# MisEty/RTG-SLAM

Measured on AMD Instinct MI355X. Metric: hot_path_units_per_sec, higher is better.
Workload: dtype f32; 1 GPU; `value` counts UNITS, not SLAM frames (the SLAM frame rate by the reference's definition is `slam_frames_per_sec`, from the `slam_sequence` leg of --full).  One UNIT per step = 1 ICP track (3 levels x 5 GN iters, 1200x680, on a second HIP stream) + 1 map-optimisation iteration (raster fwd + masked L1 colour / gated depth loss + attach regulariser + raster bwd + fused Adam) over 1200000 random Gaus; gaussians=1200000, mode=single, parallelism=1 GPU

## Files before the change

include/rtgs_debug.h:

```cpp
#ifndef RTGS_DEBUG_H
#define RTGS_DEBUG_H
#include "rtgs_raster.h"
#ifdef __cplusplus
extern "C" {
#endif

void rtgs_raster_set_counters(void* counters);
void rtgs_raster_set_counters_ctx(rtgs_ctx* ctx, void* counters);

void rtgs_raster_set_profiling(int enable);
void rtgs_raster_set_profiling_ctx(rtgs_ctx* ctx, int enable);

void rtgs_raster_set_near_slice(int mode, int budget_per_tile);
void rtgs_raster_set_near_slice_ctx(rtgs_ctx* ctx, int mode, int budget_per_tile);

void rtgs_raster_force_sort_path(int enable);
void rtgs_raster_force_sort_path_ctx(rtgs_ctx* ctx, int enable);
int rtgs_raster_last_timings(float* ms12_host);
int rtgs_raster_last_timings_ctx(rtgs_ctx* ctx, float* ms12_host);

void rtgs_raster_set_bwd_walk_ctx(rtgs_ctx* ctx, int mode);
void rtgs_raster_set_onepass_ctx(rtgs_ctx* ctx, int on);
void rtgs_raster_set_bwd_debug(int bits);
void rtgs_raster_set_bwd_stamps(void* dev);
void rtgs_raster_set_fwd_stamps(void* dev);
#define RTGS_ICP_STAMP_LAUNCHES 16
#define RTGS_ICP_STAMP_WGS 256
void rtgs_icp_set_stamps(void* dev);

#ifdef __cplusplus
}
#endif
#endif
```

rtg_slam_amd/_lib.py:

```python
from __future__ import annotations

import ctypes as C
import os
import threading

_HERE = os.path.dirname(os.path.abspath(__file__))
LIB_PATH = os.environ.get("RTGS_LIB_PATH") or os.path.join(_HERE, "librtgs_hip.so")

RESIZE_FN = C.CFUNCTYPE(C.c_void_p, C.c_void_p, C.c_size_t)
FWD_NO_BACKWARD = 1


class RasterSettingsC(C.Structure):
    _fields_ = [
        ("image_height", C.c_int32), ("image_width", C.c_int32),
        ("tanfovx", C.c_float), ("tanfovy", C.c_float),
        ("bg", C.c_void_p), ("scale_modifier", C.c_float),
        ("viewmatrix", C.c_void_p), ("projmatrix", C.c_void_p),
        ("sh_degree", C.c_int32), ("campos", C.c_void_p),
        ("opaque_threshold", C.c_float), ("depth_threshold", C.c_float),
        ("normal_threshold", C.c_float), ("color_sigma", C.c_float),
        ("prefiltered", C.c_int32), ("debug", C.c_int32),
        ("cx", C.c_float), ("cy", C.c_float), ("T_threshold", C.c_float),
    ]
# ... 93 lines not shown
    "rtgs_slam_loss_grads": (C.c_int, [_P, _P, _P, _P, _P, C.c_int32, C.c_int32, C.POINTER(LossCfgC), _P, _P, _P, _P, _P]),
    "rtgs_raster_set_profiling": (None, [C.c_int]),
    "rtgs_raster_force_sort_path": (None, [C.c_int]),
    "rtgs_raster_set_near_slice": (None, [C.c_int, C.c_int]),
    "rtgs_raster_last_slice_stats": (C.c_int, [C.POINTER(C.c_int64)]),
    "rtgs_raster_last_timings": (C.c_int, [C.POINTER(C.c_float)]),
    "rtgs_ctx_create": (C.c_void_p, []),
    "rtgs_ctx_destroy": (None, [_P]),
    "rtgs_raster_forward_ctx": (C.c_int, [_P, C.POINTER(RasterSettingsC), C.c_int32, C.c_int32] + [_P] * 6 + [_P]
                                + [_P] * 8 + [RESIZE_FN, _P, RESIZE_FN, _P, RESIZE_FN, _P, C.POINTER(C.c_int64),
                                              C.c_int32, _P]),
    "rtgs_raster_backward_ctx": (C.c_int, [_P, C.POINTER(RasterSettingsC), C.c_int32, C.c_int32, C.c_int64] + [_P] * 6
                                 + [_P] * 3 + [_P, _P, _P] + [_P, _P] + [_P] * 6 + [_P, _P]),
    "rtgs_raster_backward_rows_ctx": (C.c_int, [_P, C.POINTER(RasterSettingsC), C.c_int32, C.c_int32, C.c_int64] + [_P] * 6
                                      + [_P] * 3 + [_P, _P, _P] + [_P, _P] + [_P] * 6 + [_P, _P, _P]),
    "rtgs_raster_backward_range_ctx": (C.c_int, [_P, C.POINTER(RasterSettingsC), C.c_int32, C.c_int32, C.c_int64] + [_P] * 6
                                       + [_P] * 3 + [_P, _P, _P] + [_P, _P] + [_P] * 6 + [_P, _P, C.c_int32, C.c_int32, _P]),
    "rtgs_slam_normal_loss_range": (C.c_int, [_P, _P, _P, _P, C.c_int32, C.c_int32, C.c_float, _P, _P, _P, _P, _P,
                                              C.c_int32, C.c_int32, _P]),
    "rtgs_slam_normal_loss_sums": (C.c_int, [_P, _P, _P, _P, C.c_int32, C.c_int32, _P, _P, _P]),
    "rtgs_slam_normal_loss_grads": (C.c_int, [_P, _P, _P, _P, C.c_int32, C.c_int32, C.c_float, _P, _P, _P, _P, _P,
                                              C.c_int32, C.c_int32, _P]),
    "rtgs_raster_geom_bytes_ctx": (C.c_size_t, [_P, C.c_int32, C.c_int32, C.c_int32]),
    "rtgs_raster_last_stats_ctx": (C.c_int, [_P, C.POINTER(C.c_int64)]),
    "rtgs_raster_set_counters_ctx": (None, [_P, _P]),
    "rtgs_raster_set_profiling_ctx": (None, [_P, C.c_int]),
    "rtgs_raster_force_sort_path_ctx": (None, [_P, C.c_int]),
    "rtgs_raster_set_bwd_walk_ctx": (None, [_P, C.c_int]),
    "rtgs_raster_set_bwd_debug": (None, [C.c_int]),
    "rtgs_raster_set_bwd_stamps": (None, [C.c_void_p]),
    "rtgs_raster_set_fwd_stamps": (None, [C.c_void_p]),
    "rtgs_icp_set_stamps": (None, [C.c_void_p]),
    "rtgs_raster_set_onepass_ctx": (None, [_P, C.c_int]),
    "rtgs_raster_forward_verify_ctx": (C.c_int, [_P, C.POINTER(C.c_int64)]),
    "rtgs_raster_spec_fail_ptr_ctx": (C.c_void_p, [_P]),
    "rtgs_raster_set_speculation_ctx": (None, [_P, C.c_int]),
    "rtgs_raster_speculation_stats_ctx": (C.c_int, [_P, C.POINTER(C.c_int64)]),
    "rtgs_raster_plain_stats_ctx": (C.c_int, [_P, C.POINTER(C.c_int64)]),
    "rtgs_raster_set_plain_onepass_ctx": (None, [_P, C.c_int]),
    "rtgs_raster_image_offsets": (C.c_int, [C.c_int32, C.c_int32, C.POINTER(C.c_size_t)]),
    "rtgs_raster_set_near_slice_ctx": (None, [_P, C.c_int, C.c_int]),
    "rtgs_raster_last_slice_stats_ctx": (C.c_int, [_P, C.POINTER(C.c_int64)]),
    "rtgs_raster_last_timings_ctx": (C.c_int, [_P, C.POINTER(C.c_float)]),
    "rtgs_slam_map_step_ctx": (C.c_int, [_P, C.POINTER(MapStepArgsC), C.POINTER(C.c_int64), _P]),
    "rtgs_slam_map_step_front_ctx": (C.c_int, [_P, C.POINTER(MapStepArgsC), C.POINTER(C.c_int64), _P]),
    "rtgs_icp_build_pyramids": (C.c_int, [_P, C.c_int32, C.c_int32, _P, C.c_int32, C.POINTER(_P), C.POINTER(_P), _P, _P]),
    "rtgs_icp_build_pyramids_ex": (C.c_int, [_P, C.c_int32, C.c_int32, _P, C.c_int32, C.POINTER(_P), C.POINTER(_P), _P, C.c_int32, _P]),
    "rtgs_icp_scratch_init": (C.c_int, [_P, _P]),
    "rtgs_icp_step": (C.c_int, [_P] * 4 + [C.c_int32, C.c_int32, _P, _P, C.c_float, C.c_float, _P, _P, _P, _P, _P]),
    "rtgs_icp_track": (C.c_int, [C.POINTER(IcpLevelC), C.c_int32, _P, C.c_float, C.c_float, C.c_float, _P, _P, _P,
                                 C.c_int32, _P]),
    "rtgs_icp_fill_model_depth": (C.c_int, [_P, _P, _P, _P, C.c_int32, C.c_int32, C.c_float, C.c_float, _P]),
    "rtgs_icp_scratch_bytes": (C.c_size_t, []),
    "rtgs_tile_sum": (C.c_int, [_P, C.c_int32, C.c_int32, C.c_int32, C.c_int32, _P, _P]),
    "rtgs_transmission2tilemask": (C.c_int, [_P, C.c_int32, C.c_int32, C.c_int32, C.c_float, _P, _P, _P]),
    "rtgs_pixelmask2tilemask": (C.c_int, [_P, C.c_int32, C.c_int32, C.c_int32, _P, _P, _P]),
    "rtgs_colorerror2tilemask": (C.c_int, [_P, C.c_int32, C.c_int32, C.c_int32, C.c_float, _P, _P, _P]),
    "rtgs_colorerror2tilemask_k": (C.c_int, [_P, C.c_int32, C.c_int32, C.c_int32, C.c_int32, _P, _P, _P]),
    "rtgs_render_range": (C.c_int, [_P, C.c_int32, C.c_int32, C.c_float, _P, _P, _P, _P, _P]),
    "rtgs_knn3_scratch_bytes": (C.c_size_t, [C.c_int32]),
    "rtgs_knn3": (C.c_int, [_P, C.c_int32, _P, _P, _P, _P, _P]),
    "rtgs_knn3_query_scratch_bytes": (C.c_size_t, [C.c_int32, C.c_int32]),
    "rtgs_knn3_query": (C.c_int, [_P, C.c_int32, _P, C.c_int32, C.c_int32, _P, _P, _P, _P, _P]),
    "rtgs_knn3_built_bytes": (C.c_size_t, [C.c_int32]),
    "rtgs_knn3_query_built_scratch_bytes": (C.c_size_t, [C.c_int32]),
    "rtgs_knn3_build_ref": (C.c_int, [_P, C.c_int32, _P, _P]),
# ... 70 lines not shown
```

rtg_slam_amd/csrc/raster_api.hip:

```cpp
#include "../../include/rtgs_raster.h"
#include "../../include/rtgs_debug.h"
#include "raster_common.h"

#include <rocprim/device/device_radix_sort.hpp>
#include <rocprim/device/device_scan.hpp>
#include <math.h>
#include <new>
#include <stdlib.h>
#include <string.h>

namespace rtgs {
void launch_mask_sat(const int32_t*, int, int, int32_t*, hipStream_t);
void launch_preprocess_fwd(const RasterParams&, const float*, const float*, const float*, const float*, const float*,
                           const float*, const int32_t*, Splat*, uint32_t*, int32_t*, uint8_t*, int32_t*, uint32_t*, int,
                           uint8_t*, hipStream_t);
void launch_emit_keys(const RasterParams&, const Splat*, const int32_t*, const uint32_t*, const int32_t*, uint64_t*,
                      uint32_t*, hipStream_t);
void launch_tile_ranges(int64_t, const uint64_t*, uint2*, hipStream_t);
void set_fwd_stamps(void* dev);
void set_bwd_debug(int bits);
void set_bwd_stamps(void* dev);
void launch_blend_fwd(const RasterParams&, const uint2*, const uint32_t*, const Splat*, float*, float*, int32_t*,
                      int32_t*, float*, float*, float*, uint32_t*, unsigned long long*, SlicePass, uint32_t*, uint32_t*, uint32_t*, int, uint32_t*,
                      TileCache, uint32_t, hipStream_t);
// ... 5 lines not shown
                            const BwdInfo*, SplatGrad*, uint8_t*, const uint32_t*, uint32_t, uint32_t, TileCache, uint32_t, hipStream_t);
void launch_grad_reduce(int, const uint8_t*, const uint32_t*, uint32_t*, const BwdInfo*, SplatGrad*, const uint32_t*, hipStream_t);
void launch_preprocess_bwd(const RasterParams&, const float*, const float*, const float*, const float*, const float*,
                           const float*, const int32_t*, const uint8_t*, SplatGrad*, uint8_t*, uint8_t*, float*, float*,
                           float*, float*, float*, float*, hipStream_t);

size_t bin_lds_limit_tiles();
int bin_sort_capacity();
size_t bin_block_counts_bytes(int, int);
int launch_bin_count(const RasterParams&, const Splat*, const int32_t*, const int32_t*, uint32_t*, uint16_t*, SliceSel,
                     SliceList, size_t, hipStream_t);
size_t bin_slice_block_counts_bytes(int, size_t, int);
size_t bin_list_block_counts_bytes(int, int);
void launch_visible_compact(int, const uint8_t*, uint32_t*, uint32_t*, const uint32_t*, uint32_t*, uint32_t*, const uint32_t*, hipStream_t,
                            const SliceSel* = nullptr, int32_t* = nullptr, uint32_t* = nullptr);
void launch_slice_compact(int, SliceSel, uint32_t*, uint32_t*, const uint32_t*, uint32_t*, uint32_t*, uint32_t*, uint32_t, uint32_t*, hipStream_t);
void launch_slice_publish(int, const int32_t*, const int32_t*, const uint32_t*, uint32_t*, uint32_t*, uint32_t, uint32_t*, hipStream_t,
                          const uint32_t* seg_count = nullptr);
void launch_preprocess_cull(const RasterParams&, const float*, const float*, const float*, uint32_t*, int32_t*, int32_t*,
                            uint32_t*, int, uint8_t*, float2*, hipStream_t);
void launch_preprocess_shade(const RasterParams&, const float*, const float*, const float*, const float*, const float*,
                             const float*, Splat*, int32_t*, uint8_t*, float2*, SliceList, SliceSel, size_t, hipStream_t);
void launch_bin_tilescan(int, const uint32_t*, uint2*, uint32_t*, uint32_t*, uint32_t*, const uint32_t*, const uint32_t*,
                         const uint32_t*, const uint32_t*, uint32_t, SpecCaps, hipStream_t);
void launch_bin_scatter(const RasterParams&, const Splat*, const int32_t*, const int32_t*, const uint16_t*, uint32_t*,
                        unsigned long long*, SliceSel, SliceList, size_t, hipStream_t);
void launch_slice_hist(int, const uint8_t*, const uint32_t*, const int32_t*, uint32_t*, unsigned long long*, hipStream_t,
                       BwdInfoInit bi = BwdInfoInit{nullptr, nullptr, 0u, 0u});
void launch_bin_tilesort(int, uint32_t, const uint2*, const unsigned long long*, uint32_t*, const uint32_t*, hipStream_t,
                         const uint32_t* seg_count = nullptr, uint32_t seg = 0, uint2* ranges_out = nullptr,
                         const BinFinish* finish = nullptr);
void launch_bin_place(const RasterParams&, const Splat*, const int32_t*, const int32_t*, uint32_t*, unsigned long long*, uint32_t,
                      uint32_t*, SliceSel, SliceList, size_t, hipStream_t);

}

enum { EV_F0 = 0, EV_PRE, EV_SL_BIN, EV_SL_BLEND, EV_SCAN, EV_BIN0, EV_EMIT, EV_SORT, EV_RANGES, EV_BLEND0, EV_BLEND, EV_B0,
       EV_BWALK, EV_BBLEND, EV_BPRE, EV_N };
struct rtgs_ctx {
  int64_t stats[8] = {0};
  int slice_mode = 2;
  int slice_budget = 384;
  int64_t slice_stats[4] = {0};
  unsigned long long* counters = nullptr;
  uint32_t last_listed = 0;
  bool onepass = true;
  bool prof = false;
  bool force_sort_path = false;
  int bwd_walk = 0;
  bool ev_init = false;
  hipEvent_t ev[EV_N];
  bool ev_set[EV_N] = {false};
  uint32_t* info_host = nullptr;
  uint32_t seq = 0;
  const void* hint_geom = nullptr;
  bool hint_slice_lists = true, hint_main_lists = true;
  int hint_walk = -2;
  void *last_geom = nullptr, *last_bin = nullptr, *last_img = nullptr;
  uint32_t* aux_zero = nullptr;
  bool ask_first = false;
  struct Plan {
    bool valid = false;
    int32_t P = 0, H = 0, W = 0;
    int kind = -1;
    int slice_mode = 0, slice_budget = 0;
    uint32_t R = 0, R1 = 0, longest = 0, slots = 0, n_fin = 0;
    uint32_t R_hi = 0, longest_hi = 0, slots_hi = 0;
    void note(uint32_t r, uint32_t l, uint32_t s) {
      R = r; longest = l; slots = s;
      R_hi = r > R_hi - R_hi / 16 ? r : R_hi - R_hi / 16;
      longest_hi = l > longest_hi - longest_hi / 16 ? l : longest_hi - longest_hi / 16;
      slots_hi = s > slots_hi - slots_hi / 16 ? s : slots_hi - slots_hi / 16;
    }
  } plan;
  struct Spec {
    bool pending = false;
    int kind = -1;
    uint32_t seq = 0, capR = 0, capL = 0, capS = 0;
    const void* geom = nullptr;
    const uint32_t* fail_dev = nullptr;
    void* stream = nullptr;
    int32_t ntiles = 0;
    int64_t G_total = 0, B_total = 0, I_total = 0;
  } spec;
  bool speculation = true;
  int64_t spec_stats[3] = {0, 0, 0};
  Plan plan_plain;
  Plan plan_plain0;
  bool plain_onepass = true;
  int64_t plain_stats[2] = {0, 0};
};

namespace rtgs {

static rtgs_ctx* default_ctx() {
  static rtgs_ctx* c = [] {
    rtgs_ctx* n = new rtgs_ctx();
    if (const char* e = getenv("RTGS_NEAR_SLICE")) n->slice_mode = atoi(e);
    if (const char* e = getenv("RTGS_NEAR_SLICE_BUDGET")) { const int b = atoi(e); if (b > 0) n->slice_budget = b; }
    if (const char* e = getenv("RTGS_SPECULATE")) n->speculation = atoi(e) != 0;
    if (const char* e = getenv("RTGS_BIN_ONEPASS")) n->onepass = atoi(e) != 0;
    if (const char* e = getenv("RTGS_PLAIN_ONEPASS")) n->plain_onepass = atoi(e) != 0;
    if (const char* e = getenv("RTGS_BWD_WALK")) { const int m = atoi(e); n->bwd_walk = (m >= 1 && m <= 4) ? m : 0; }
    return n;
  }();
  return c;
}
static inline rtgs_ctx* use(rtgs_ctx* c) { return c ? c : default_ctx(); }

static void prof_mark(rtgs_ctx* c, int which, hipStream_t st) {
  if (!c->prof) return;
  if (!c->ev_init) {
    for (int i = 0; i < EV_N; ++i) (void)hipEventCreate(&c->ev[i]);
    c->ev_init = true;
  }
  (void)hipEventRecord(c->ev[which], st);
  c->ev_set[which] = true;
}

static int bits_for(uint32_t n) {
  int b = 0;
  while ((1ull << b) < (unsigned long long)n) ++b;
  return b < 1 ? 1 : b;
}

static int wait_published_words(uint32_t* info_host, uint32_t seq, hipStream_t st, uint32_t (&pub)[7]) {
  volatile uint32_t* h = info_host;
  auto snapshot_ok = [&]() -> bool {
    if (h[7] != seq) return false;
    __atomic_thread_fence(__ATOMIC_ACQUIRE);
    uint32_t w[7];
    for (int k = 0; k < 7; ++k) w[k] = h[k];
    if (h[8] != host_checksum(seq, w)) return false;
    for (int k = 0; k < 7; ++k) pub[k] = w[k];
    return true;
// ... 136 lines not shown
  p.spec_fail = nullptr;
  return RTGS_OK;
}

#define HIP_TRY(expr)                         \
  do {                                        \
    hipError_t e_ = (expr);                   \
    if (e_ != hipSuccess) return RTGS_E_HIP;  \
  } while (0)

static int dbg_sync(const rtgs_raster_settings* s, hipStream_t st) {
  if (s->debug) {
    HIP_TRY(hipStreamSynchronize(st));
    HIP_TRY(hipGetLastError());
  }
  return RTGS_OK;
}
#define DBG(s, st)                              \
  do {                                          \
    int r_ = dbg_sync(s, st);                   \
    if (r_ != RTGS_OK) return r_;               \
  } while (0)

}

using namespace rtgs;

extern "C" {

const char* rtgs_version(void) { return "rtgs-hip 0.2.0 (gfx950)"; }

rtgs_ctx* rtgs_ctx_create(void) {
  rtgs_ctx* c = new (std::nothrow) rtgs_ctx();
  if (c) { c->slice_mode = default_ctx()->slice_mode; c->slice_budget = default_ctx()->slice_budget; c->bwd_walk = default_ctx()->bwd_walk; c->onepass = default_ctx()->onepass; c->speculation = default_ctx()->speculation; c->plain_onepass = default_ctx()->plain_onepass; }
  return c;
}
void rtgs_ctx_destroy(rtgs_ctx* c) {
  if (!c || c == default_ctx()) return;
  if (c->ev_init) for (int i = 0; i < EV_N; ++i) (void)hipEventDestroy(c->ev[i]);
  if (c->info_host) (void)hipHostFree(c->info_host);
  delete c;
}

size_t rtgs_raster_geom_bytes_ctx(rtgs_ctx* c, int32_t P, int32_t H, int32_t W) {
  return geom_layout(P, (W + TILE - 1) / TILE, (H + TILE - 1) / TILE, use(c)->slice_budget).total;
}
size_t rtgs_raster_geom_bytes(int32_t P, int32_t H, int32_t W) { return rtgs_raster_geom_bytes_ctx(nullptr, P, H, W); }
size_t rtgs_raster_binning_bytes(int64_t R, int32_t H, int32_t W) {
  const int gx = (W + TILE - 1) / TILE, gy = (H + TILE - 1) / TILE;
  return bin_layout(R, gx * gy, true, 0).total;
}
size_t rtgs_raster_image_bytes(int32_t H, int32_t W) {
  const int gx = (W + TILE - 1) / TILE, gy = (H + TILE - 1) / TILE;
  return img_layout(H, W, gx * gy).total;
}
size_t rtgs_raster_backward_scratch_bytes(int32_t P) {
  const size_t n = (size_t)(P > 0 ? P : 1);
  return align_up(n * sizeof(SplatGrad)) + align_up(n);
}

int rtgs_raster_last_stats_ctx(rtgs_ctx* c, int64_t* out) {
  if (!out) return RTGS_E_INVALID;
  memcpy(out, use(c)->stats, sizeof(use(c)->stats));
  return RTGS_OK;
}
void rtgs_raster_set_counters_ctx(rtgs_ctx* c, void* counters) { use(c)->counters = (unsigned long long*)counters; }

// ... 96 lines not shown
                           pl.slice_budget == c->slice_budget && (pl.kind == 0 ? !sliced : (pl.kind == 1 || pl.kind == 2) && sliced));
    const uint32_t capR = pl.R_hi + pl.R_hi / 8u + 8192u, capL = sort_class_cap(pl.longest_hi),
                   capS = immediate ? 0u : pl.slots_hi + pl.slots_hi / 8u + 8192u;
    if ((flags & RTGS_FWD_SPECULATE) && !(eligible && (pl.kind == 1 || capS <= SLOTS_MAX))) ++c->spec_stats[2];
    if (eligible && (pl.kind == 1 || capS <= SLOTS_MAX)) {
      uint32_t* const fail = slice_ctr + 6;
      const SliceSel sel1{1, zbin, slice_hist, (uint32_t)G.slice_cap, (uint32_t)G.slice_max_list, slice_ctr, nullptr, nullptr,
                          slice_cover, (uint32_t)ntiles * (uint32_t)(TILE * TILE), slice_auto ? 1 : 0};
      const SpecCaps nocaps{nullptr, 0u, 0u, 0u, nullptr};
      if (++c->seq == 0u) c->seq = 1u;
      size_t b_total = 0;
      bool seg_main = false;
      if (pl.kind == 1) {
        launch_preprocess_cull(p, means3D, scales, rotations, tiles_touched, radii, out_radii, zero_words, zero_n, zbin,
                               (float2*)(geom + G.uv), st);
        prof_mark(c, EV_PRE, st);
        const uint32_t sl = (uint32_t)G.slice_cap;
        const bool use_sl = sl > 0 && sl <= SLOTS_MAX;
        const BinLayout B = bin_layout(0, ntiles, false, use_sl ? (size_t)sl : 0);
        char* bin = (char*)binning_resize(binning_user, B.total);
        if (!bin) return RTGS_E_ALLOC;
        c->last_bin = bin;
        b_total = B.total;
        launch_slice_hist(P, zbin, tiles_touched, radii, slice_hist, slice_cover, st,
                          BwdInfoInit{(BwdInfo*)(img + I.bwd_info), (SplatGrad*)(bin + B.slot_grads), use_sl ? sl : 0u, use_sl ? 1u : 0u});
        launch_slice_compact(P, sel1, (uint32_t*)(geom + G.slice_ids), slice_ctr + 2, tiles_touched, offsets, slice_ctr + 4,
                             nullptr, 0u, nullptr, st);
        const SliceList work{(const uint32_t*)(geom + G.slice_ids), slice_ctr + 2};
        launch_preprocess_shade(p, means3D, opacities, shs, scales, rotations, normal_w, splats, radii, clamped,
                                (float2*)(geom + G.uv), work, sel1, G.slice_max_list, st);
        if (seg1) {
          launch_bin_place(p, splats, radii, tile_mask, tile_count1, (unsigned long long*)(geom + G.bucket1), seg1, nullptr,
                           sel1, work, G.slice_max_list, st);
          launch_bin_tilesort(ntiles, (uint32_t)SLICE_MAX_LIST, ranges1, (const unsigned long long*)(geom + G.bucket1), list1,
                              nullptr, st, tile_count1, seg1, ranges1);
        } else {
        if (launch_bin_count(p, splats, radii, tile_mask, tile_count1, (uint16_t*)(geom + G.block_counts1), sel1, work,
                             G.slice_max_list, st) != 0)
          return RTGS_E_HIP;
        launch_bin_tilescan(ntiles, tile_count1, ranges1, (uint32_t*)(geom + G.cursor1), info + 2, nullptr, nullptr,
                            nullptr, nullptr, nullptr, 0u, nocaps, st);
        launch_bin_scatter(p, splats, radii, tile_mask, (const uint16_t*)(geom + G.block_counts1),
                           (uint32_t*)(geom + G.cursor1), (unsigned long long*)(geom + G.bucket1), sel1, work,
                           G.slice_max_list, st);
        launch_bin_tilesort(ntiles, (uint32_t)SLICE_MAX_LIST, ranges1, (const unsigned long long*)(geom + G.bucket1), list1,
                            nullptr, st);
        }
        prof_mark(c, EV_SL_BIN, st);
        const SlicePass pass1{1, tile_mask, mask2, ranges1_bwd, ranges};
        launch_blend_fwd(p, ranges1, list1, splats, out_color, out_depth, out_cidx, out_didx, out_cw, out_dw, out_T,
                         n_contrib, c->counters, pass1, tile_mode, depth_pos, tile_last, fwd_walk, aux_zero, tcache, seg1, st);
        prof_mark(c, EV_SL_BLEND, st);
        launch_slice_publish(ntiles, tile_mask, mask2, info + 2, slice_ctr, info_host, c->seq, fail, st, seg1 ? tile_count1 : nullptr);
        prof_mark(c, EV_BLEND0, st); prof_mark(c, EV_BLEND, st);
        c->hint_slice_lists = true; c->hint_main_lists = false;
        c->slice_stats[0] = 1; c->slice_stats[1] = pl.R1; c->slice_stats[2] = pl.n_fin; c->slice_stats[3] = 0;
      } else {
        const uint32_t seg2 = (c->onepass && ((pl.kind == 2 && G.slice_seg) || (immediate && pl.kind == 0))) ? capL : 0u;
        const BinLayout B = bin_layout(seg2 ? (int64_t)ntiles * (int64_t)seg2 : (int64_t)capR, ntiles, false, (size_t)capS);
        seg_main = seg2 != 0u;
        char* bin = (char*)binning_resize(binning_user, B.total);
        if (!bin) return RTGS_E_ALLOC;
        c->last_bin = bin;
        b_total = B.total;
        RasterParams pg = p;
        pg.spec_fail = fail;
        SliceList vl{nullptr, nullptr};
        if (pl.kind == 2) {
// ... 95 lines not shown
      if (!sort_path && want_bwd && (rc = scan_all()) != RTGS_OK) return rc;
    } else {
      launch_preprocess_cull(p, means3D, scales, rotations, tiles_touched, radii, out_radii, zero_words, zero_n, zbin,
                             (float2*)(geom + G.uv), st);
    }
    DBG(s, st);
    prof_mark(c, EV_PRE, st);
    if (sliced) {
      launch_slice_hist(P, zbin, tiles_touched, radii, slice_hist, slice_cover, st);
      const bool ask = slice_auto && c->ask_first;
      if (ask && ++c->seq == 0u) c->seq = 1u;
      launch_slice_compact(P, sel1, (uint32_t*)(geom + G.slice_ids), slice_ctr + 2, tiles_touched, offsets, slice_ctr + 4,
                           ask ? info_host : nullptr, c->seq, nullptr, st);
      if (ask) {
        if ((rc = wait_published(c->seq)) != RTGS_OK) return rc;
        declined = (int32_t)pub[6] < 0;
      }
    }
    if (sliced && declined) {
      vis = SliceList{(const uint32_t*)(geom + G.vis_ids), slice_ctr + 4};
      launch_visible_compact(P, zbin, (uint32_t*)(geom + G.vis_ids), slice_ctr + 4, tiles_touched, offsets, slice_ctr + 5, nullptr, st);
      launch_preprocess_shade(p, means3D, opacities, shs, scales, rotations, normal_w, splats, radii, clamped,
                              (float2*)(geom + G.uv), vis, sel1, (size_t)P, st);
      sliced = false;
      considered = true;
    }
    if (sliced) {
      const SliceList work{(const uint32_t*)(geom + G.slice_ids), slice_ctr + 2};
      launch_preprocess_shade(p, means3D, opacities, shs, scales, rotations, normal_w, splats, radii, clamped,
                              (float2*)(geom + G.uv), work, sel1, G.slice_max_list, st);
      if (seg1) {
        launch_bin_place(p, splats, radii, tile_mask, tile_count1, (unsigned long long*)(geom + G.bucket1), seg1, nullptr,
                         sel1, work, G.slice_max_list, st);
        launch_bin_tilesort(ntiles, (uint32_t)SLICE_MAX_LIST, ranges1, (const unsigned long long*)(geom + G.bucket1), list1,
                            nullptr, st, tile_count1, seg1, ranges1);
      } else {
      if (launch_bin_count(p, splats, radii, tile_mask, tile_count1, (uint16_t*)(geom + G.block_counts1), sel1, work,
                           G.slice_max_list, st) != 0)
        return RTGS_E_HIP;
      launch_bin_tilescan(ntiles, tile_count1, ranges1, (uint32_t*)(geom + G.cursor1), info + 2, nullptr, nullptr,
                          nullptr, nullptr, nullptr, 0u, SpecCaps{nullptr, 0u, 0u, 0u, nullptr}, st);
      launch_bin_scatter(p, splats, radii, tile_mask, (const uint16_t*)(geom + G.block_counts1),
                         (uint32_t*)(geom + G.cursor1), (unsigned long long*)(geom + G.bucket1), sel1, work,
                         G.slice_max_list, st);
      launch_bin_tilesort(ntiles, (uint32_t)SLICE_MAX_LIST, ranges1, (const unsigned long long*)(geom + G.bucket1), list1,
                          nullptr, st);
      }
      DBG(s, st);
      prof_mark(c, EV_SL_BIN, st);
      if (++c->seq == 0u) c->seq = 1u;
      const SlicePass pass1{1, tile_mask, mask2, ranges1_bwd, ranges};
      launch_blend_fwd(p, ranges1, list1, splats, out_color, out_depth, out_cidx, out_didx, out_cw, out_dw, out_T,
                       n_contrib, c->counters, pass1, tile_mode, depth_pos, tile_last, fwd_walk, aux_zero, tcache, seg1, st);
      prof_mark(c, EV_SL_BLEND, st);
      launch_slice_publish(ntiles, tile_mask, mask2, info + 2, slice_ctr, info_host, c->seq, nullptr, st, seg1 ? tile_count1 : nullptr);
      DBG(s, st);
      if ((rc = wait_published(c->seq)) != RTGS_OK) return rc;
      n_left = pub[2]; n_fin = pub[3];
      R1 = (int64_t)pub[4];
      if (n_left > 0) {
        mask_main = mask2;
        pass = SlicePass{2, nullptr, mask2, nullptr, nullptr};
        launch_mask_sat(mask2, p.gx, p.gy, sat, st);
        SliceSel sel_rest = sel1;
        sel_rest.sat = sat; sel_rest.uv = (const float2*)(geom + G.uv);
        launch_preprocess_shade(p, means3D, opacities, shs, scales, rotations, normal_w, splats, radii, clamped,
                                (float2*)(geom + G.uv), SliceList{nullptr, nullptr}, sel_rest, 0, st);
        if (want_bwd && (rc = scan_all()) != RTGS_OK) return rc;
// ... 284 lines not shown
  if (!ok) { pl.valid = false; ++c->spec_stats[1]; }
  return ok ? 0 : 1;
}
const uint32_t* rtgs_raster_spec_fail_ptr_ctx(rtgs_ctx* ctx) {
  rtgs_ctx* c = use(ctx);
  return c->spec.pending ? c->spec.fail_dev : nullptr;
}
void rtgs_raster_set_speculation_ctx(rtgs_ctx* ctx, int enable) {
  rtgs_ctx* c = use(ctx);
  c->speculation = enable != 0;
  c->plan = rtgs_ctx::Plan();
}
int rtgs_raster_speculation_stats_ctx(rtgs_ctx* ctx, int64_t* out3) {
  if (!out3) return RTGS_E_INVALID;
  memcpy(out3, use(ctx)->spec_stats, sizeof(use(ctx)->spec_stats));
  return RTGS_OK;
}
int rtgs_raster_plain_stats_ctx(rtgs_ctx* ctx, int64_t* out2) {
  if (!out2) return RTGS_E_INVALID;
  memcpy(out2, use(ctx)->plain_stats, sizeof(use(ctx)->plain_stats));
  return RTGS_OK;
}
void rtgs_raster_set_plain_onepass_ctx(rtgs_ctx* ctx, int enable) {
  rtgs_ctx* c = use(ctx);
  c->plain_onepass = enable != 0;
  c->plan_plain = rtgs_ctx::Plan();
  c->plan_plain0 = rtgs_ctx::Plan();
}
uint32_t rtgs_raster_last_listed_ctx(rtgs_ctx* c) { return use(c)->last_listed; }
void rtgs_raster_set_bwd_debug(int bits) { rtgs::set_bwd_debug(bits); }
void rtgs_raster_set_bwd_stamps(void* dev) { rtgs::set_bwd_stamps(dev); }
void rtgs_raster_set_fwd_stamps(void* dev) { rtgs::set_fwd_stamps(dev); }
void rtgs_raster_set_onepass_ctx(rtgs_ctx* c, int on) { use(c)->onepass = on != 0; use(c)->plan.valid = false; }
void rtgs_raster_set_bwd_walk_ctx(rtgs_ctx* c, int mode) { use(c)->bwd_walk = (mode >= 1 && mode <= 4) ? mode : 0; }
void rtgs_raster_set_aux_zero_ctx(rtgs_ctx* ctx, void* eight_words) { use(ctx)->aux_zero = (uint32_t*)eight_words; }
int rtgs_raster_last_buffers_ctx(rtgs_ctx* ctx, void** out3) {
  rtgs_ctx* c = use(ctx);
  if (!out3 || !c->last_geom || !c->last_bin || !c->last_img) return RTGS_E_INVALID;
  out3[0] = c->last_geom; out3[1] = c->last_bin; out3[2] = c->last_img;
  return RTGS_OK;
}
int rtgs_raster_backward_buffers(int32_t P, int32_t H, int32_t W, size_t* out) {
  if (!out || P < 0 || H <= 0 || W <= 0) return RTGS_E_INVALID;
  const int gx = (W + TILE - 1) / TILE, gy = (H + TILE - 1) / TILE;
  const GeomLayout G = geom_layout(P, gx, gy, 1);
  const ImgLayout I = img_layout(H, W, gx * gy);
  out[0] = G.clamped; out[1] = G.offsets; out[2] = G.slot_count; out[3] = I.bwd_info;
  out[4] = align_up((size_t)(P > 0 ? P : 1) * sizeof(SplatGrad)); out[5] = G.radii; out[6] = 0; out[7] = 0;
  return RTGS_OK;
}
int rtgs_raster_image_offsets(int32_t H, int32_t W, size_t* out) {
  if (!out || H <= 0 || W <= 0) return RTGS_E_INVALID;
  const int gx = (W + TILE - 1) / TILE, gy = (H + TILE - 1) / TILE;
  const ImgLayout I = img_layout(H, W, gx * gy);
  out[0] = I.ranges; out[1] = I.n_contrib; out[2] = I.bwd_info; out[3] = I.tile_mode; out[4] = I.total; out[5] = I.depth_pos;
  return RTGS_OK;
}

int rtgs_raster_last_timings_ctx(rtgs_ctx* ctx, float* ms) {
  rtgs_ctx* c = use(ctx);
  if (!ms) return RTGS_E_INVALID;
  for (int i = 0; i < 12; ++i) ms[i] = -1.f;
  if (!c->ev_init) return RTGS_OK;
  const int pre_end = c->ev_set[EV_SL_BLEND] ? EV_SL_BLEND : EV_PRE;
  const int pairs[11][2] = {{EV_F0, EV_PRE}, {pre_end, EV_SCAN}, {EV_BIN0, EV_EMIT}, {EV_EMIT, EV_SORT},
                            {EV_SORT, EV_RANGES}, {EV_BLEND0, EV_BLEND}, {EV_B0, EV_BWALK}, {EV_BBLEND, EV_BPRE},
// ... 56 lines not shown
```

rtg_slam_amd/csrc/raster_bin.hip:

```cpp
#include "raster_common.h"
#include <mutex>

namespace rtgs {

struct LdsGrant {
  std::mutex m;
  size_t got[64];
  explicit LdsGrant(size_t base) { for (size_t& g : got) g = base; }
  void ensure(const void* fn, size_t lds) {
    int dev = 0;
    (void)hipGetDevice(&dev);
    if (dev < 0 || dev >= 64) { (void)hipFuncSetAttribute(fn, hipFuncAttributeMaxDynamicSharedMemorySize, (int)lds); return; }
    std::lock_guard<std::mutex> lk(m);
    if (lds > got[dev]) {
      (void)hipFuncSetAttribute(fn, hipFuncAttributeMaxDynamicSharedMemorySize, (int)lds);
      got[dev] = lds;
    }
  }
};

constexpr int GPB = 1024;
#ifndef RTGS_SLICE_GPB
#define RTGS_SLICE_GPB 32
#endif
// ... 339 lines not shown
__global__ void __launch_bounds__(THREADS) bin_tilesort_kernel(const uint2* __restrict__ ranges,
                                                               const unsigned long long* __restrict__ bucket,
                                                               uint32_t* __restrict__ point_list, int lo, int hi,
                                                               const uint32_t* __restrict__ spec_fail, TileSeg ts,
                                                               BinFinish fin) {
  extern __shared__ unsigned long long s_key[];
  if (fin.count && (int)blockIdx.x == fin.ntiles) { bin_finish(fin); return; }
  if (spec_failed(spec_fail)) return;
  const uint2 r = tile_range(ranges, ts, threadIdx.x == 0);
  const int n = (int)(r.y - r.x);
  if (n < lo || n >= hi) return;
  const int tid = threadIdx.x;
  if (n == 1) { if (tid == 0) point_list[r.x] = (uint32_t)bucket[r.x]; return; }
  int n2 = 2;
  while (n2 < n) n2 <<= 1;
  for (int i = tid; i < n2; i += THREADS) s_key[i] = (i < n) ? bucket[r.x + i] : ~0ull;
  __syncthreads();
  for (int k = 2; k <= n2; k <<= 1) {
    for (int j = k >> 1; j > 0; j >>= 1) {
      for (int i = tid; i < (n2 >> 1); i += THREADS) {
        const int a = ((i & ~(j - 1)) << 1) | (i & (j - 1));
        const int b = a | j;
        const unsigned long long ka = s_key[a], kb = s_key[b];
        const bool up = (a & k) == 0;
        if ((ka > kb) == up) { s_key[a] = kb; s_key[b] = ka; }
      }
      __syncthreads();
    }
  }
  for (int i = tid; i < n; i += THREADS) point_list[r.x + i] = (uint32_t)s_key[i];
}

template <int THREADS>
__global__ void __launch_bounds__(THREADS) bin_tilesort_radix_kernel(const uint2* __restrict__ ranges,
                                                                     const unsigned long long* __restrict__ bucket,
                                                                     uint32_t* __restrict__ point_list, int lo, int hi,
                                                                     int cap, const uint32_t* __restrict__ spec_fail,
                                                                     TileSeg ts) {
  constexpr int NW = THREADS / 64;
  extern __shared__ unsigned long long s_dyn[];
  unsigned long long* kA = s_dyn;
  unsigned long long* kB = s_dyn + cap;
  uint32_t* s_cnt = reinterpret_cast<uint32_t*>(s_dyn + 2 * cap);
  uint32_t* s_tot = s_cnt + NW * 256;
  __shared__ uint32_t s_or;
  if (spec_failed(spec_fail)) return;
  const uint2 r = tile_range(ranges, ts, false);
  const int n = (int)(r.y - r.x);
  if (n < lo || n >= hi) return;
  const int tid = threadIdx.x, lane = tid & 63, w = tid >> 6;
  if (tid == 0) s_or = 0;
  __syncthreads();
  const uint32_t z0 = (uint32_t)(bucket[r.x] >> 32);
  uint32_t vary = 0;
  for (int i = tid; i < n; i += THREADS) {
    const unsigned long long k = bucket[r.x + i];
    kA[i] = k;
    vary |= (uint32_t)(k >> 32) ^ z0;
  }
#pragma unroll
  for (int off = 32; off > 0; off >>= 1) vary |= (uint32_t)__shfl_xor((int)vary, off);
  if (lane == 0 && vary) atomicOr(&s_or, vary);
  __syncthreads();
  const uint32_t vbits = s_or;
  const int seg = ((n + NW - 1) / NW + 63) & ~63;
  const int wlo = min(n, w * seg), whi = min(n, wlo + seg);
  for (int pass = 0; pass < 4; ++pass) {
    if (((vbits >> (8 * pass)) & 0xffu) == 0) continue;
    const int shift = 32 + 8 * pass;
    for (int i = tid; i < NW * 256; i += THREADS) s_cnt[i] = 0;
    __syncthreads();
    for (int i = wlo + lane; i < whi; i += 64) atomicAdd(&s_cnt[w * 256 + (int)((kA[i] >> shift) & 0xff)], 1u);
    __syncthreads();
    if (tid < 256) {
      uint32_t run = 0;
#pragma unroll
      for (int ww = 0; ww < NW; ++ww) { const uint32_t c = s_cnt[ww * 256 + tid]; s_cnt[ww * 256 + tid] = run; run += c; }
      s_tot[tid] = run;
    }
    __syncthreads();
    if (tid < 64) {
      uint32_t v0 = s_tot[4 * tid], v1 = s_tot[4 * tid + 1], v2 = s_tot[4 * tid + 2], v3 = s_tot[4 * tid + 3];
// ... 23 lines not shown
        const unsigned long long below = same & ((1ull << lane) - 1ull);
        const uint32_t base = s_cnt[w * 256 + d] + s_tot[d];
        kB[base + (uint32_t)__popcll(below)] = k;
        if ((same >> lane) == 1ull) s_cnt[w * 256 + d] += (uint32_t)__popcll(same);
      }
    }
    __syncthreads();
    unsigned long long* tmp = kA; kA = kB; kB = tmp;
  }
  bool tie = false;
  for (int i = tid + 1; i < n; i += THREADS) tie |= (uint32_t)(kA[i] >> 32) == (uint32_t)(kA[i - 1] >> 32);
  if (__syncthreads_or(tie)) {
    for (int i = tid; i < n; i += THREADS) {
      const unsigned long long key = kA[i];
      const uint32_t z = (uint32_t)(key >> 32);
      int lo = 0, hi = i;
      while (lo < hi) { const int mid = (lo + hi) >> 1; if ((uint32_t)(kA[mid] >> 32) < z) lo = mid + 1; else hi = mid; }
      const int first = lo;
      lo = i; hi = n;
      while (lo < hi) { const int mid = (lo + hi) >> 1; if ((uint32_t)(kA[mid] >> 32) <= z) lo = mid + 1; else hi = mid; }
      int rank = first;
      if (lo - first > 1)
        for (int j = first; j < lo; ++j) rank += (kA[j] < key) ? 1 : 0;
      else
        rank = i;
      kB[rank] = key;
    }
    __syncthreads();
    unsigned long long* tmp = kA; kA = kB; kB = tmp;
  }
  for (int i = tid; i < n; i += THREADS) point_list[r.x + i] = (uint32_t)kA[i];
}

size_t bin_lds_limit_tiles() { return 16000; }
int bin_sort_capacity() { return 16384; }

#ifndef RTGS_LIST_GPB
#define RTGS_LIST_GPB 256
#endif
constexpr int LIST_GPB = RTGS_LIST_GPB;
static inline int list_gpb(const SliceList& list, size_t max_items) {
  return !list.ids ? GPB : (max_items > 65536 ? LIST_GPB : SLICE_GPB);
}
size_t bin_list_block_counts_bytes(int P, int ntiles) {
  const size_t rows = P > 65536 ? ((size_t)P + LIST_GPB - 1) / LIST_GPB : ((size_t)P + SLICE_GPB - 1) / SLICE_GPB;
  return rows * (size_t)ntiles * sizeof(uint16_t);
}
size_t bin_block_counts_bytes(int P, int ntiles) {
  return (size_t)((P + GPB - 1) / GPB) * (size_t)ntiles * sizeof(uint16_t);
}
size_t bin_slice_block_counts_bytes(int P, size_t max_list, int ntiles) {
  const size_t n = max_list < (size_t)P ? max_list : (size_t)P;
  return ((n + SLICE_GPB - 1) / SLICE_GPB) * (size_t)ntiles * sizeof(uint16_t);
}

__global__ void __launch_bounds__(256) slice_hist_kernel(int P, const uint8_t* __restrict__ zbin,
                                                         const uint32_t* __restrict__ rect_area,
                                                         const int32_t* __restrict__ radii,
                                                         uint32_t* __restrict__ hist,
                                                         unsigned long long* __restrict__ cover, BwdInfoInit bi) {
  __shared__ uint32_t s_h[SLICE_BINS], s_c[SLICE_BINS], s_r[SLICE_BINS];
  if (bi.dst && blockIdx.x == 0 && threadIdx.x == 0) {
    bi.dst->slot_grads = bi.slot_grads; bi.dst->slots = bi.slots; bi.dst->use_slots = bi.use_slots;
  }
  s_h[threadIdx.x] = 0; s_c[threadIdx.x] = 0; s_r[threadIdx.x] = 0;
  __syncthreads();
// ... 241 lines not shown
  const size_t n = list.ids && max_items < (size_t)p.P ? max_items : (size_t)p.P;
  hipLaunchKernelGGL(bin_scatter_kernel, dim3((unsigned)((n + gpb - 1) / gpb)), dim3(BLOCK), lds, st, p, splats, radii,
                     mask, block_counts, cursor, bucket, sel, list, gpb);
}
void launch_bin_place(const RasterParams& p, const Splat* splats, const int32_t* radii, const int32_t* mask,
                      uint32_t* seg_count, unsigned long long* bucket, uint32_t seg, uint32_t* fail, SliceSel sel,
                      SliceList list, size_t max_items, hipStream_t st) {
  if (p.P == 0) return;
  const int ntiles = p.gx * p.gy;
  const size_t lds = (size_t)ntiles * sizeof(uint32_t);
  static LdsGrant grant(24 * 1024);
  grant.ensure((const void*)bin_place_kernel, lds);
  static const int stage_cap = [] { const char* e = getenv("RTGS_BIN_STAGE"); const int v = e ? atoi(e) : STAGE_W;
                                    return v < 0 ? 0 : (v > STAGE_W ? STAGE_W : v); }();
  const int gpb = list_gpb(list, max_items);
  const size_t n = max_items < (size_t)p.P ? max_items : (size_t)p.P;
  const int stage = (list.ids != nullptr && gpb <= BLOCK && ntiles < 16384) ? stage_cap : 0;
  hipLaunchKernelGGL(bin_place_kernel, dim3((unsigned)((n + gpb - 1) / gpb)), dim3(BLOCK), lds, st, p, splats, radii, mask,
                     SegBins{seg_count, bucket, seg, fail}, sel, list, gpb, stage);
}

template <int THREADS>
static void launch_radix(int ntiles, const uint2* ranges, const unsigned long long* bucket, uint32_t* point_list, int lo,
                         int hi, int cap, const uint32_t* spec_fail, TileSeg ts, hipStream_t st) {
  const size_t lds = (size_t)cap * 16 + (size_t)(THREADS / 64 + 1) * 256 * sizeof(uint32_t);
  static LdsGrant grant(48 * 1024);
  grant.ensure((const void*)bin_tilesort_radix_kernel<THREADS>, lds);
  hipLaunchKernelGGL(bin_tilesort_radix_kernel<THREADS>, dim3(ntiles), dim3(THREADS), lds, st, ranges, bucket, point_list,
                     lo, hi, cap, spec_fail, ts);
}

void launch_bin_tilesort(int ntiles, uint32_t longest, const uint2* ranges, const unsigned long long* bucket,
                         uint32_t* point_list, const uint32_t* spec_fail, hipStream_t st, const uint32_t* seg_count,
                         uint32_t seg, uint2* ranges_out, const BinFinish* finish) {
  const TileSeg ts{seg_count, seg, nullptr}, ts0{seg_count, seg, ranges_out};
  const BinFinish nofin{nullptr, 0, nullptr, nullptr, nullptr, nullptr, nullptr, 0u, SpecCaps{nullptr, 0u, 0u, 0u, nullptr}};
  const BinFinish fin = finish ? *finish : nofin;
  hipLaunchKernelGGL(bin_tilesort_kernel<128>, dim3(ntiles + (fin.count ? 1 : 0)), dim3(128), 256 * 8, st, ranges, bucket, point_list,
                     1, 257, spec_fail, ts0, fin);
  if (longest > 256) launch_radix<256>(ntiles, ranges, bucket, point_list, 257, 1025, 1024, spec_fail, ts, st);
  if (longest > 1024) launch_radix<512>(ntiles, ranges, bucket, point_list, 1025, 3073, 3072, spec_fail, ts, st);
  if (longest > 3072) launch_radix<1024>(ntiles, ranges, bucket, point_list, 3073, 8193, 8192, spec_fail, ts, st);
  if (longest > 8192) {
    static LdsGrant grant(48 * 1024);
    grant.ensure((const void*)bin_tilesort_kernel<1024>, 16384 * 8);
    hipLaunchKernelGGL(bin_tilesort_kernel<1024>, dim3(ntiles), dim3(1024), 16384 * 8, st, ranges, bucket, point_list,
                       8193, 16385, spec_fail, ts, nofin);
  }
}

}
```

rtg_slam_amd/rasterizer.py:

```python
from __future__ import annotations

import ctypes as C
import threading
from typing import NamedTuple, Optional

import torch
import torch.nn as nn

from . import _lib


class GaussianRasterizationSettings(NamedTuple):
    image_height: int
    image_width: int
    tanfovx: float
    tanfovy: float
    bg: torch.Tensor
    scale_modifier: float
    viewmatrix: torch.Tensor
    projmatrix: torch.Tensor
    sh_degree: int
    campos: torch.Tensor
    opaque_threshold: float
    depth_threshold: float
# ... 12 lines not shown
        self.handle = handle
        self._owned = owned

    @classmethod
    def create(cls) -> "RasterContext":
        h = _lib.load().rtgs_ctx_create()
        if not h:
            raise RuntimeError("rtgs_ctx_create failed")
        return cls(h, owned=True)

    def __del__(self):
        try:
            if self._owned and self.handle:
                _lib.load().rtgs_ctx_destroy(C.c_void_p(self.handle))
                self.handle = None
        except Exception:
            pass

    @property
    def ptr(self):
        return C.c_void_p(self.handle)

    def set_near_slice(self, mode: int, budget_per_tile: int = 0):
        _lib.load().rtgs_raster_set_near_slice_ctx(self.ptr, int(mode), int(budget_per_tile))

    def force_sort_path(self, enable: bool):
        _lib.load().rtgs_raster_force_sort_path_ctx(self.ptr, int(bool(enable)))

    def set_bwd_walk(self, mode: int):
        _lib.load().rtgs_raster_set_bwd_walk_ctx(self.ptr, int(mode))

    def set_onepass(self, enable: bool):
        _lib.load().rtgs_raster_set_onepass_ctx(self.ptr, int(bool(enable)))

    def set_speculation(self, enable: bool):
        _lib.load().rtgs_raster_set_speculation_ctx(self.ptr, int(bool(enable)))

    def speculation_stats(self):
        out = (C.c_int64 * 3)()
        _lib.check(_lib.load().rtgs_raster_speculation_stats_ctx(self.ptr, out), "rtgs_raster_speculation_stats")
        return dict(speculative=int(out[0]), failed=int(out[1]), not_eligible=int(out[2]))

    def set_plain_onepass(self, enable: bool):
        _lib.load().rtgs_raster_set_plain_onepass_ctx(self.ptr, int(bool(enable)))

    def plain_stats(self):
        out = (C.c_int64 * 2)()
        _lib.check(_lib.load().rtgs_raster_plain_stats_ctx(self.ptr, out), "rtgs_raster_plain_stats")
        return dict(onepass=int(out[0]), redone=int(out[1]))

    def set_profiling(self, enable: bool):
        _lib.load().rtgs_raster_set_profiling_ctx(self.ptr, int(bool(enable)))

    def set_counters(self, counters: Optional[torch.Tensor]):
        _lib.load().rtgs_raster_set_counters_ctx(self.ptr, C.c_void_p(counters.data_ptr() if counters is not None else 0))

    def last_stats(self):
        out = (C.c_int64 * 8)()
        _lib.check(_lib.load().rtgs_raster_last_stats_ctx(self.ptr, out), "rtgs_raster_last_stats")
        return [int(v) for v in out]

    def last_slice_stats(self):
        out = (C.c_int64 * 4)()
        _lib.check(_lib.load().rtgs_raster_last_slice_stats_ctx(self.ptr, out), "rtgs_raster_last_slice_stats")
        return dict(used=int(out[0]), instances=int(out[1]), tiles_finished=int(out[2]), tiles_left_to_pass2=int(out[3]))

# ... 270 lines not shown
```

Before: 2656 units/s.

## Sort near-slice tile lists with one wave per tile and in-kernel radix fallback

Adds a single-launch slice tilesort kernel where each wavefront sorts one tile's near-slice key list. It uses an in-register bitonic sort for lists up to 1024 keys, and longer lists fall back to a block-wide LDS radix sort inside the same kernel. This replaces the cascade of size-bucketed tilesort launches, each of which scans all tiles, for the slice path. It is enabled by default through a new per-context flag. The cost is a large LDS allocation per block, and a block containing one long list serialises its radix sort behind the short ones.

```diff
diff --git a/include/rtgs_debug.h b/include/rtgs_debug.h
--- a/include/rtgs_debug.h
+++ b/include/rtgs_debug.h
@@ -21,6 +21,7 @@
 
 void rtgs_raster_set_bwd_walk_ctx(rtgs_ctx* ctx, int mode);
 void rtgs_raster_set_onepass_ctx(rtgs_ctx* ctx, int on);
+void rtgs_raster_set_slice_front_ctx(rtgs_ctx* ctx, int on);
 void rtgs_raster_set_bwd_debug(int bits);
 void rtgs_raster_set_bwd_stamps(void* dev);
 void rtgs_raster_set_fwd_stamps(void* dev);
diff --git a/rtg_slam_amd/_lib.py b/rtg_slam_amd/_lib.py
--- a/rtg_slam_amd/_lib.py
+++ b/rtg_slam_amd/_lib.py
@@ -149,6 +149,7 @@
     "rtgs_raster_set_fwd_stamps": (None, [C.c_void_p]),
     "rtgs_icp_set_stamps": (None, [C.c_void_p]),
     "rtgs_raster_set_onepass_ctx": (None, [_P, C.c_int]),
+    "rtgs_raster_set_slice_front_ctx": (None, [_P, C.c_int]),
     "rtgs_raster_forward_verify_ctx": (C.c_int, [_P, C.POINTER(C.c_int64)]),
     "rtgs_raster_spec_fail_ptr_ctx": (C.c_void_p, [_P]),
     "rtgs_raster_set_speculation_ctx": (None, [_P, C.c_int]),
diff --git a/rtg_slam_amd/csrc/raster_api.hip b/rtg_slam_amd/csrc/raster_api.hip
--- a/rtg_slam_amd/csrc/raster_api.hip
+++ b/rtg_slam_amd/csrc/raster_api.hip
@@ -61,6 +61,8 @@
                          const BinFinish* finish = nullptr);
 void launch_bin_place(const RasterParams&, const Splat*, const int32_t*, const int32_t*, uint32_t*, unsigned long long*, uint32_t,
                       uint32_t*, SliceSel, SliceList, size_t, hipStream_t);
+void launch_bin_tilesort_slice(int, const unsigned long long*, uint32_t*, const uint32_t*, const uint32_t*, uint32_t, uint2*,
+                               hipStream_t);
 
 }
 
@@ -117,6 +119,7 @@
   Plan plan_plain;
   Plan plan_plain0;
   bool plain_onepass = true;
+  bool slice_front = true;
   int64_t plain_stats[2] = {0, 0};
 };
 
@@ -130,6 +133,7 @@
     if (const char* e = getenv("RTGS_SPECULATE")) n->speculation = atoi(e) != 0;
     if (const char* e = getenv("RTGS_BIN_ONEPASS")) n->onepass = atoi(e) != 0;
     if (const char* e = getenv("RTGS_PLAIN_ONEPASS")) n->plain_onepass = atoi(e) != 0;
+    if (const char* e = getenv("RTGS_SLICE_FRONT")) n->slice_front = atoi(e) != 0;
     if (const char* e = getenv("RTGS_BWD_WALK")) { const int m = atoi(e); n->bwd_walk = (m >= 1 && m <= 4) ? m : 0; }
     return n;
   }();
@@ -332,7 +336,7 @@
 
 rtgs_ctx* rtgs_ctx_create(void) {
   rtgs_ctx* c = new (std::nothrow) rtgs_ctx();
-  if (c) { c->slice_mode = default_ctx()->slice_mode; c->slice_budget = default_ctx()->slice_budget; c->bwd_walk = default_ctx()->bwd_walk; c->onepass = default_ctx()->onepass; c->speculation = default_ctx()->speculation; c->plain_onepass = default_ctx()->plain_onepass; }
+  if (c) { c->slice_mode = default_ctx()->slice_mode; c->slice_budget = default_ctx()->slice_budget; c->bwd_walk = default_ctx()->bwd_walk; c->onepass = default_ctx()->onepass; c->speculation = default_ctx()->speculation; c->plain_onepass = default_ctx()->plain_onepass; c->slice_front = default_ctx()->slice_front; }
   return c;
 }
 void rtgs_ctx_destroy(rtgs_ctx* c) {
@@ -495,8 +499,12 @@
         if (seg1) {
           launch_bin_place(p, splats, radii, tile_mask, tile_count1, (unsigned long long*)(geom + G.bucket1), seg1, nullptr,
                            sel1, work, G.slice_max_list, st);
-          launch_bin_tilesort(ntiles, (uint32_t)SLICE_MAX_LIST, ranges1, (const unsigned long long*)(geom + G.bucket1), list1,
-                              nullptr, st, tile_count1, seg1, ranges1);
+          if (c->slice_front)
+            launch_bin_tilesort_slice(ntiles, (const unsigned long long*)(geom + G.bucket1), list1, nullptr, tile_count1, seg1,
+                                      ranges1, st);
+          else
+            launch_bin_tilesort(ntiles, (uint32_t)SLICE_MAX_LIST, ranges1, (const unsigned long long*)(geom + G.bucket1), list1,
+                                nullptr, st, tile_count1, seg1, ranges1);
         } else {
         if (launch_bin_count(p, splats, radii, tile_mask, tile_count1, (uint16_t*)(geom + G.block_counts1), sel1, work,
                              G.slice_max_list, st) != 0)
@@ -658,8 +666,12 @@
       if (seg1) {
         launch_bin_place(p, splats, radii, tile_mask, tile_count1, (unsigned long long*)(geom + G.bucket1), seg1, nullptr,
                          sel1, work, G.slice_max_list, st);
-        launch_bin_tilesort(ntiles, (uint32_t)SLICE_MAX_LIST, ranges1, (const unsigned long long*)(geom + G.bucket1), list1,
-                            nullptr, st, tile_count1, seg1, ranges1);
+        if (c->slice_front)
+          launch_bin_tilesort_slice(ntiles, (const unsigned long long*)(geom + G.bucket1), list1, nullptr, tile_count1, seg1,
+                                    ranges1, st);
+        else
+          launch_bin_tilesort(ntiles, (uint32_t)SLICE_MAX_LIST, ranges1, (const unsigned long long*)(geom + G.bucket1), list1,
+                              nullptr, st, tile_count1, seg1, ranges1);
       } else {
       if (launch_bin_count(p, splats, radii, tile_mask, tile_count1, (uint16_t*)(geom + G.block_counts1), sel1, work,
                            G.slice_max_list, st) != 0)
@@ -1010,6 +1022,7 @@
 void rtgs_raster_set_bwd_stamps(void* dev) { rtgs::set_bwd_stamps(dev); }
 void rtgs_raster_set_fwd_stamps(void* dev) { rtgs::set_fwd_stamps(dev); }
 void rtgs_raster_set_onepass_ctx(rtgs_ctx* c, int on) { use(c)->onepass = on != 0; use(c)->plan.valid = false; }
+void rtgs_raster_set_slice_front_ctx(rtgs_ctx* c, int on) { use(c)->slice_front = on != 0; }
 void rtgs_raster_set_bwd_walk_ctx(rtgs_ctx* c, int mode) { use(c)->bwd_walk = (mode >= 1 && mode <= 4) ? mode : 0; }
 void rtgs_raster_set_aux_zero_ctx(rtgs_ctx* ctx, void* eight_words) { use(ctx)->aux_zero = (uint32_t*)eight_words; }
 int rtgs_raster_last_buffers_ctx(rtgs_ctx* ctx, void** out3) {
diff --git a/rtg_slam_amd/csrc/raster_bin.hip b/rtg_slam_amd/csrc/raster_bin.hip
--- a/rtg_slam_amd/csrc/raster_bin.hip
+++ b/rtg_slam_amd/csrc/raster_bin.hip
@@ -395,22 +395,14 @@
 }
 
 template <int THREADS>
-__global__ void __launch_bounds__(THREADS) bin_tilesort_radix_kernel(const uint2* __restrict__ ranges,
-                                                                     const unsigned long long* __restrict__ bucket,
-                                                                     uint32_t* __restrict__ point_list, int lo, int hi,
-                                                                     int cap, const uint32_t* __restrict__ spec_fail,
-                                                                     TileSeg ts) {
+__device__ __forceinline__ void radix_sort_tile(uint2 r, int n, const unsigned long long* __restrict__ bucket,
+                                                uint32_t* __restrict__ point_list, int cap, unsigned long long* s_dyn,
+                                                uint32_t& s_or) {
   constexpr int NW = THREADS / 64;
-  extern __shared__ unsigned long long s_dyn[];
   unsigned long long* kA = s_dyn;
   unsigned long long* kB = s_dyn + cap;
   uint32_t* s_cnt = reinterpret_cast<uint32_t*>(s_dyn + 2 * cap);
   uint32_t* s_tot = s_cnt + NW * 256;
-  __shared__ uint32_t s_or;
-  if (spec_failed(spec_fail)) return;
-  const uint2 r = tile_range(ranges, ts, false);
-  const int n = (int)(r.y - r.x);
-  if (n < lo || n >= hi) return;
   const int tid = threadIdx.x, lane = tid & 63, w = tid >> 6;
   if (tid == 0) s_or = 0;
   __syncthreads();
@@ -500,6 +492,123 @@
   for (int i = tid; i < n; i += THREADS) point_list[r.x + i] = (uint32_t)kA[i];
 }
 
+template <int THREADS>
+__global__ void __launch_bounds__(THREADS) bin_tilesort_radix_kernel(const uint2* __restrict__ ranges,
+                                                                     const unsigned long long* __restrict__ bucket,
+                                                                     uint32_t* __restrict__ point_list, int lo, int hi,
+                                                                     int cap, const uint32_t* __restrict__ spec_fail,
+                                                                     TileSeg ts) {
+  extern __shared__ unsigned long long s_dyn[];
+  __shared__ uint32_t s_or;
+  if (spec_failed(spec_fail)) return;
+  const uint2 r = tile_range(ranges, ts, false);
+  const int n = (int)(r.y - r.x);
+  if (n < lo || n >= hi) return;
+  radix_sort_tile<THREADS>(r, n, bucket, point_list, cap, s_dyn, s_or);
+}
+
+constexpr int SORT1_W = 8;
+constexpr int WAVE_SORT_MAX = 1024;
+constexpr int SORT1_THREADS = SORT1_W * 64;
+
+__device__ __forceinline__ unsigned long long shfl_xor_u64(unsigned long long v, int m) {
+  const int lo = __shfl_xor((int)(uint32_t)v, m), hi = __shfl_xor((int)(uint32_t)(v >> 32), m);
+  return ((unsigned long long)(uint32_t)hi << 32) | (uint32_t)lo;
+}
+
+template <int KPL>
+__device__ __forceinline__ void wave_bitonic(unsigned long long (&k)[KPL], int n2, int lane) {
+  const int e0 = lane * KPL;
+  for (int kk = 2; kk <= n2; kk <<= 1) {
+    for (int j = kk >> 1; j >= KPL; j >>= 1) {
+      const bool up = (e0 & kk) == 0, lower = (e0 & j) == 0;
+      const bool keep_min = lower == up;
+#pragma unroll
+      for (int q = 0; q < KPL; ++q) {
+        const unsigned long long o = shfl_xor_u64(k[q], j / KPL);
+        const bool lt = o < k[q];
+        k[q] = (lt == keep_min) ? o : k[q];
+      }
+    }
+#pragma unroll
+    for (int j = KPL / 2; j >= 1; j >>= 1) {
+      if (j >= kk) continue;
+#pragma unroll
+      for (int q = 0; q < KPL; ++q) {
+        if (q & j) continue;
+        const bool up = ((e0 + q) & kk) == 0;
+        const unsigned long long a = k[q], b = k[q | j];
+        if ((a > b) == up) { k[q] = b; k[q | j] = a; }
+      }
+    }
+  }
+}
+
+template <int KPL>
+__device__ __forceinline__ void wave_sort_list(const unsigned long long* __restrict__ bucket, uint32_t* __restrict__ point_list,
+                                               uint32_t x0, int n, int lane) {
+  const int e0 = lane * KPL;
+  unsigned long long k[KPL];
+  if (e0 + KPL <= n) {
+#pragma unroll
+    for (int q = 0; q < KPL; q += 2) {
+      const ulonglong2 a = *reinterpret_cast<const ulonglong2*>(bucket + x0 + e0 + q);
+      k[q] = a.x; k[q + 1] = a.y;
+    }
+  } else {
+#pragma unroll
+    for (int q = 0; q < KPL; ++q) k[q] = e0 + q < n ? bucket[x0 + e0 + q] : ~0ull;
+  }
+  int n2 = 2;
+  while (n2 < n) n2 <<= 1;
+  wave_bitonic<KPL>(k, n2, lane);
+  if (e0 + KPL <= n) {
+#pragma unroll
+    for (int q = 0; q < KPL; q += 4)
+      *reinterpret_cast<uint4*>(point_list + x0 + e0 + q) = make_uint4((uint32_t)k[q], (uint32_t)k[q + 1], (uint32_t)k[q + 2], (uint32_t)k[q + 3]);
+  } else {
+#pragma unroll
+    for (int q = 0; q < KPL; ++q) if (e0 + q < n) point_list[x0 + e0 + q] = (uint32_t)k[q];
+  }
+}
+
+__global__ void __launch_bounds__(SORT1_THREADS) bin_tilesort_slice_kernel(const unsigned long long* __restrict__ bucket,
+                                                                          uint32_t* __restrict__ point_list,
+                                                                          const uint32_t* __restrict__ spec_fail,
+                                                                          const uint32_t* __restrict__ count, uint32_t seg,
+                                                                          uint2* __restrict__ ranges_out, int ntiles) {
+  extern __shared__ unsigned long long s_dyn[];
+  __shared__ uint32_t s_or, s_long[SORT1_W];
+  if (spec_failed(spec_fail)) return;
+  const int lane = threadIdx.x & 63, w = threadIdx.x >> 6;
+  const int t = blockIdx.x + w * gridDim.x;
+  int n = 0;
+  uint32_t x0 = 0;
+  if (t < ntiles) {
+    x0 = (uint32_t)t * seg;
+    n = (int)count[t];
+    if (lane == 0 && ranges_out) ranges_out[t] = make_uint2(x0, x0 + (uint32_t)n);
+  }
+  const int cap = min((int)seg, SLICE_MAX_LIST);
+  if (lane == 0) s_long[w] = (n > WAVE_SORT_MAX && n <= cap) ? (uint32_t)n : 0u;
+  if (n == 1) {
+    if (lane == 0) point_list[x0] = (uint32_t)bucket[x0];
+  } else if (n >= 2 && n <= 256) {
+    wave_sort_list<4>(bucket, point_list, x0, n, lane);
+  } else if (n > 256 && n <= WAVE_SORT_MAX && n <= cap) {
+    if (n <= 512) wave_sort_list<8>(bucket, point_list, x0, n, lane);
+    else wave_sort_list<16>(bucket, point_list, x0, n, lane);
+  }
+  __syncthreads();
+  for (int v = 0; v < SORT1_W; ++v) {
+    const int nl = (int)s_long[v];
+    if (nl == 0) continue;
+    const uint32_t xl = (uint32_t)(blockIdx.x + v * gridDim.x) * seg;
+    radix_sort_tile<SORT1_THREADS>(make_uint2(xl, xl + (uint32_t)nl), nl, bucket, point_list, SLICE_MAX_LIST, s_dyn, s_or);
+    __syncthreads();
+  }
+}
+
 size_t bin_lds_limit_tiles() { return 16000; }
 int bin_sort_capacity() { return 16384; }
 
@@ -807,6 +916,23 @@
 
 void launch_bin_tilesort(int ntiles, uint32_t longest, const uint2* ranges, const unsigned long long* bucket,
                          uint32_t* point_list, const uint32_t* spec_fail, hipStream_t st, const uint32_t* seg_count,
+                         uint32_t seg, uint2* ranges_out, const BinFinish* finish = nullptr);
+void launch_bin_tilesort_slice(int ntiles, const unsigned long long* bucket, uint32_t* point_list, const uint32_t* spec_fail,
+                               const uint32_t* seg_count, uint32_t seg, uint2* ranges_out, hipStream_t st) {
+  if (ntiles <= 0) return;
+  if (seg % 4u != 0u || seg > (uint32_t)SLICE_MAX_LIST) {
+    launch_bin_tilesort(ntiles, (uint32_t)SLICE_MAX_LIST, nullptr, bucket, point_list, spec_fail, st, seg_count, seg, ranges_out);
+    return;
+  }
+  const size_t lds = (size_t)SLICE_MAX_LIST * 16 + (size_t)(SORT1_W + 1) * 256 * sizeof(uint32_t);
+  static LdsGrant grant(48 * 1024);
+  grant.ensure((const void*)bin_tilesort_slice_kernel, lds);
+  hipLaunchKernelGGL(bin_tilesort_slice_kernel, dim3((unsigned)((ntiles + SORT1_W - 1) / SORT1_W)), dim3(SORT1_THREADS), lds, st,
+                     bucket, point_list, spec_fail, seg_count, seg, ranges_out, ntiles);
+}
+
+void launch_bin_tilesort(int ntiles, uint32_t longest, const uint2* ranges, const unsigned long long* bucket,
+                         uint32_t* point_list, const uint32_t* spec_fail, hipStream_t st, const uint32_t* seg_count,
                          uint32_t seg, uint2* ranges_out, const BinFinish* finish) {
   const TileSeg ts{seg_count, seg, nullptr}, ts0{seg_count, seg, ranges_out};
   const BinFinish nofin{nullptr, 0, nullptr, nullptr, nullptr, nullptr, nullptr, 0u, SpecCaps{nullptr, 0u, 0u, 0u, nullptr}};
diff --git a/rtg_slam_amd/rasterizer.py b/rtg_slam_amd/rasterizer.py
--- a/rtg_slam_amd/rasterizer.py
+++ b/rtg_slam_amd/rasterizer.py
@@ -68,6 +68,9 @@
 
     def set_onepass(self, enable: bool):
         _lib.load().rtgs_raster_set_onepass_ctx(self.ptr, int(bool(enable)))
+
+    def set_slice_front(self, enable: bool):
+        _lib.load().rtgs_raster_set_slice_front_ctx(self.ptr, int(bool(enable)))
 
     def set_speculation(self, enable: bool):
         _lib.load().rtgs_raster_set_speculation_ctx(self.ptr, int(bool(enable)))
```

Result: faster. 2724 units/s, median of 6 (+2.6%).
